# boycehbz/MvSMPLfitting

Hardware: AMD Instinct MI355X
Metric: L-BFGS closure evaluations per second (fwd+bwd, all concurrently fitted problems), 8-view 1-person 4-stage fits (higher is better)
Workload: dtype f32

## Files before the change

### mvsmplfitting_amd/csrc/closure_device.h

```cpp
#pragma once
#include <cstddef>
#include "mvfit_device.h"

namespace mvfit {

struct ObsBlock {
    float camR[MVFIT_MAX_VIEWS][9];
    float camt[MVFIT_MAX_VIEWS][3];
    float camf[MVFIT_MAX_VIEWS];
    float camc[MVFIT_MAX_VIEWS][2];
    float gt[MVFIT_MAX_VIEWS * NKP * 2];
    float wc[MVFIT_MAX_VIEWS * NKP];
    float gt3d[NKP * 3];
    float c3d[NKP];
};
struct PoseBlock {
    float theta[72];
    float R[NJ][9];
    float rod[NJ][3];
    float J[NJ][3];
    float Mj[32][12];
    float G[NJ][12];
    float A[NJ][12];
};
// ... 684 lines not shown
    for (int k = 0, item = own.first; k < own.n; ++k, item += FWD_THREADS) {
        float4 v[FWD_RPS];
        fwd_item_load(M, nc_pad, item, v);
        __builtin_amdgcn_sched_barrier(0);
        fwd_item_fma(L, nc_pad, item, v);
    }
}

__device__ __forceinline__ void keypoints_from_xs(ClosureLds& L, int tid) {
    if (tid < NKP * 3) {
        const int k = tid / 3, a = tid - 3 * k;
        float acc = 0.f;
        if (L.M.padded) {
            int si[KP_NZ];
            float wi[KP_NZ], xv[KP_NZ];
#pragma unroll
            for (int t = 0; t < KP_NZ; ++t) { si[t] = L.M.kpp_s[k][t]; wi[t] = L.M.kpp_w[k][t]; }
#pragma unroll
            for (int t = 0; t < KP_NZ; ++t) xv[t] = L.xs[3 * si[t] + a];
#pragma unroll
            for (int t = 0; t < KP_NZ; ++t) acc = fmaf(wi[t], xv[t], acc);
        } else {
            for (int t = L.M.kp_start[k]; t < L.M.kp_start[k + 1]; ++t) acc = fmaf(L.M.kp_w[t], L.xs[3 * L.M.kp_s[t] + a], acc);
        }
        if (L.M.n_skel) {
            const int j = kp_joint_of(L.M, k);
            if (j >= 0) acc = L.pose.G[j][4 * a + 3];
        }
        L.kp[k][a] = acc + L.opt.x[X_TR + a];
    }
    __syncthreads();
}

__device__ __forceinline__ void sparse_forward(const DevModel& M, ClosureLds& L, bool from_pass, int tid, bool run_chain, const FwdEarly& ev) {
    const int nc = L.M.nc, nc_pad = L.M.nc_pad;
    const int nks = fwd_slices(nc_pad, STEP_NT - 64);
    if (run_chain || !from_pass) {
        const long long t_e2 = PH_CLK();
        const int wave_t0 = __builtin_amdgcn_readfirstlane(tid);
        if (ev.wave) {
            const FwdOwner own = fwd_item_owner(nc_pad, tid - 64);
            if (own.early) fwd_item_fma(L, nc_pad, own.first, ev.v);
        }
        if (wave_t0 == 0) {
            if (run_chain) chain_forward_wave(L, tid);
            PH_T(22);
        } else if (!from_pass && !ev.wave) {
            __builtin_assume(tid >= 64);
            contraction_forward(M, L, tid - 64);
        }
        PH_W(60, 64, t_e2); PH_W(62, 448, t_e2);
        __syncthreads();
    }
    PH_T(1);
    if (tid < nc) {
        const int c = tid, s = c / 3, a = c - 3 * s;
        float4 tr = make_float4(0.f, 0.f, 0.f, 0.f);
        if (L.M.sel_sparse) {
            const float4 w4 = *reinterpret_cast<const float4*>(L.M.selw[s]);
            const unsigned jj = L.M.selj[s];
            const float wv[4] = {w4.x, w4.y, w4.z, w4.w};
            float4 av[4];
#pragma unroll
            for (int t = 0; t < 4; ++t) av[t] = *reinterpret_cast<const float4*>(&L.pose.A[(jj >> (8 * t)) & 255u][4 * a]);
#pragma unroll
            for (int t = 0; t < 4; ++t) {
                tr.x = fmaf(wv[t], av[t].x, tr.x); tr.y = fmaf(wv[t], av[t].y, tr.y);
                tr.z = fmaf(wv[t], av[t].z, tr.z); tr.w = fmaf(wv[t], av[t].w, tr.w);
            }
        } else {
#pragma unroll 8
            for (int j = 0; j < NJ; ++j) {
                const float w = L.M.wT[j][s];
                const float4 av = *reinterpret_cast<const float4*>(&L.pose.A[j][4 * a]);
                tr.x = fmaf(w, av.x, tr.x); tr.y = fmaf(w, av.y, tr.y);
                tr.z = fmaf(w, av.z, tr.z); tr.w = fmaf(w, av.w, tr.w);
            }
        }
        *reinterpret_cast<float4*>(&L.T[s][4 * a]) = tr;
        if (!from_pass) {
            float vp[3];
#pragma unroll
            for (int b = 0; b < 3; ++b) {
                float v = L.M.vt_sub[3 * s + b];
                for (int k = 0; k < nks; ++k) v += L.scratch[k * nc_pad + 3 * s + b];
                vp[b] = v;
            }
            L.vposed[c] = vp[a];
            L.xs[c] = tr.x * vp[0] + tr.y * vp[1] + tr.z * vp[2] + tr.w;
        }
    }
    __syncthreads();
    keypoints_from_xs(L, tid);
}
__device__ __forceinline__ void sparse_forward(const DevModel& M, ClosureLds& L, bool from_pass, int tid, bool run_chain = true) {
    FwdEarly none;
    sparse_forward(M, L, from_pass, tid, run_chain, none);
}

template <bool SDFW = false, bool SDFT = true>
__device__ __forceinline__ double loss_combine(const DevModel& M, ClosureLds& L, int V, const DevWeights& W, bool writer) {
    const bool use_vp = (W.flags & MVFIT_F_VPOSER) != 0;
    const bool use_gmm = !use_vp && (W.flags & MVFIT_F_PRIOR_GMM);
    const int ndw = (V * NKP + 63) >> 6;
    double l_data = 0.0;
    for (int w = 0; w < ndw; ++w) l_data += L.red_d[w];
    const bool use_3d = (W.flags & MVFIT_F_USE_3D) != 0;
    if (use_3d) l_data += L.red_d[STEP_NW];
    l_data *= (double)W.data_w2;
    const double sq = L.red_d[STEP_NW - 1], sqb = L.red_d[STEP_NW - 2], san = L.red_d[STEP_NW - 3];
    const double wp2 = (double)W.pose_w * (double)W.pose_w;
    double l_pose;
    int dropped = 0;
    if (use_vp) {
        l_pose = sq * wp2;
    } else {
        double P;
        if (use_gmm) {
            int sel = 0;
            float best = L.gmm_ll[0];
            for (int m = 1; m < M.gmm_M; ++m) if (L.gmm_ll[m] < best) { best = L.gmm_ll[m]; sel = m; }
            if (writer) L.gmm_sel = sel;
            P = (double)best;
        } else {
            P = sq;
        }
        P *= wp2;
        if ((float)P > 5e4f) { P = 0.0; dropped |= 1; }
        l_pose = P + sq * (16.0 * wp2);
    }
// ... 6 lines not shown
    if (SDFT && L.sdf_adj && W.coll_w > 0.f) {
        bool answered = true;
        if constexpr (SDFW) {
            if (L.sdf_wait_tag) {
                if (!L.sh_sdf_ok) answered = false;
                else {
                    const long long t0 = wall_clock64();
                    while (__hip_atomic_load(L.sdf_wait_tag, __ATOMIC_RELAXED, __HIP_MEMORY_SCOPE_AGENT) < L.sdf_wait_want) {
                        if (wall_clock64() - t0 > 20000000) { answered = false; break; }
                        __builtin_amdgcn_s_sleep(8);
                    }
                    if (!answered && writer) { atomicAdd(L.sdf_wait_stats, 1u); L.sh_sdf_ok = 0u; }
                }
            }
        }
        const float S = answered ? sdf_ld(&L.sdf_adj->S) : __builtin_nanf("");
        const double ws = (double)W.coll_w * (double)S;
        l_coll = ws * ws;
        sdf_fac = 2.f * W.coll_w * W.coll_w * S;
    }
    const double total = l_data + l_pose + l_shape + l_angle + l_coll;
    if (writer) {
        L.sdf_fac = sdf_fac;
        L.loss_terms[0] = (float)l_data; L.loss_terms[1] = (float)l_pose; L.loss_terms[2] = (float)l_shape;
        L.loss_terms[3] = (float)l_angle; L.loss_terms[4] = (float)l_coll; L.loss_terms[5] = (float)total;
        L.flags_dropped = dropped;
        L.total = total;
    }
    return total;
}

template <bool DEFER = false>
__device__ __forceinline__ double loss_and_keypoint_grad(const DevModel& M, ClosureLds& L, int V, const DevWeights& W,
                                         bool want_grad, int tid) {
    const bool use_vp = (W.flags & MVFIT_F_VPOSER) != 0;
    const bool use_gmm = !use_vp && (W.flags & MVFIT_F_PRIOR_GMM);
    const int wave = tid >> 6;
    const int ndata = V * NKP;
    const int ndw = (ndata + 63) >> 6;
    double part = 0.0;
    float g0 = 0.f, g1 = 0.f, g2 = 0.f;
    if (tid < ndata) {
        const int v = tid / NKP, k = tid - v * NKP;
        const float X = L.kp[k][0], Y = L.kp[k][1], Z = L.kp[k][2];
        const float* Rc = L.obs.camR[v];
        const float* tc = L.obs.camt[v];
        const float f = L.obs.camf[v];
        const float cx = L.obs.camc[v][0], cy = L.obs.camc[v][1];
        const float px = Rc[0] * X + Rc[1] * Y + Rc[2] * Z + tc[0];
        const float py = Rc[3] * X + Rc[4] * Y + Rc[5] * Z + tc[1];
        const float pz = Rc[6] * X + Rc[7] * Y + Rc[8] * Z + tc[2];
        const float ipz = 1.0f / pz;
        const float u = f * (px * ipz) + cx, w_ = f * (py * ipz) + cy;
        const float rx = L.obs.gt[tid * 2] - u, ry = L.obs.gt[tid * 2 + 1] - w_;
        const float wcf = L.obs.wc[tid];
        const float w2 = wcf * wcf;
        const float rx2 = rx * rx, ry2 = ry * ry;
        const float idx = 1.0f / (rx2 + W.rho2), idy = 1.0f / (ry2 + W.rho2);
        const float gmx = W.rho2 * (rx2 * idx), gmy = W.rho2 * (ry2 * idy);
        part = (double)(w2 * (gmx + gmy));
        if (want_grad) {
            const float gu = -w2 * W.data_w2 * (2.f * rx * W.rho2 * W.rho2 * (idx * idx));
            const float gv = -w2 * W.data_w2 * (2.f * ry * W.rho2 * W.rho2 * (idy * idy));
            const float gpx = f * gu * ipz, gpy = f * gv * ipz;
            const float gpz = -f * (gu * px + gv * py) * (ipz * ipz);
            g0 = Rc[0] * gpx + Rc[3] * gpy + Rc[6] * gpz;
            g1 = Rc[1] * gpx + Rc[4] * gpy + Rc[7] * gpz;
            g2 = Rc[2] * gpx + Rc[5] * gpy + Rc[8] * gpz;
            L.gkp_part[v][k][0] = g0; L.gkp_part[v][k][1] = g1; L.gkp_part[v][k][2] = g2;
        }
    }
    if (wave < ndw) {
        const double pd = wave64_sum(part);
        if ((tid & 63) == 0) L.red_d[wave] = pd;
        if (want_grad) {
            const float s0 = wave64_sum(g0), s1 = wave64_sum(g1), s2 = wave64_sum(g2);
            if ((tid & 63) == 0) { L.red_f[wave][0] = s0; L.red_f[wave][1] = s1; L.red_f[wave][2] = s2; }
        }
    } else if (wave == STEP_NW - 3 && (W.flags & MVFIT_F_USE_3D)) {
        const int lane = tid & 63;
        double p3 = 0.0;
        if (lane < NKP * 3) {
            const int k = lane / 3;
            const float r = L.obs.gt3d[lane] - (&L.kp[0][0])[lane];
            const float c2 = L.obs.c3d[k] * L.obs.c3d[k];
            const float id = 1.0f / (r * r + W.rho2);
            p3 = (double)(c2 * (W.rho2 * (r * r * id)));
            if (want_grad) (&L.gkp3[0][0])[lane] = -c2 * W.data_w2 * (2.f * r * W.rho2 * W.rho2 * (id * id));
        }
        const double s3 = wave64_sum(p3);
        if (lane == 0) L.red_d[STEP_NW] = s3;
    } else if (wave == STEP_NW - 1) {
        const int lane = tid & 63;
        double pp = 0.0, bb = 0.0, an = 0.0;
        if (use_vp) { if (lane < 32) { const double v = (double)L.opt.x[X_EMB + lane]; pp = v * v; } }
        else {
            { const double v = (double)L.pose.theta[3 + lane]; pp = v * v; }
            if (lane < 5) { const double v = (double)L.pose.theta[3 + 64 + lane]; pp += v * v; }
        }
        if (lane < 10) { const double v = (double)L.opt.x[X_BETAS + lane]; bb = v * v; }
        if (lane < 4) {
            const int idx = lane == 0 ? 52 : lane == 1 ? 55 : lane == 2 ? 9 : 12;
            const float sg = lane == 0 ? 1.f : -1.f;
            const float e0 = expf(sg * L.pose.theta[3 + idx]);
            an = (double)(e0 * e0);
        }
        const double spp = wave64_sum(pp), sbb = wave64_sum(bb), san = wave64_sum(an);
        if (lane == 0) { L.red_d[STEP_NW - 1] = spp; L.red_d[STEP_NW - 2] = sbb; L.red_d[STEP_NW - 3] = san; }
    }
    if (use_gmm) {
        const int Mg = M.gmm_M;
        __syncthreads();
        float* dm = L.scratch;
        for (int i = tid; i < Mg * 72; i += STEP_NT) {
            const int m = i / 72, c = i - 72 * m;
            dm[i] = c < 69 ? L.pose.theta[3 + c] - M.gmm_means[m * 69 + c] : 0.f;
        }
// ... 150 lines not shown
__device__ __forceinline__ void bwd_item_load(const DevModel& M, int nc_pad, int item, float4 (&v)[BWD_CPS]) {
    constexpr int npq = KROWS >> 2;
    const int cps = ((nc_pad >> 2) + BWD_SLICES - 1) / BWD_SLICES * 4;
    const int pq = item % npq, cs = (item / npq + (int)blockIdx.x) & (BWD_SLICES - 1);
    const int c0 = cs * cps;
    const float4* src = reinterpret_cast<const float4*>(M.pd_subT) + pq;
#pragma unroll
    for (int r = 0; r < BWD_CPS; ++r) {
        const int c = min(c0 + r, nc_pad - 1);
        if (r < BWD_SMPL_CPS || r < cps) v[r] = src[(size_t)c * npq];
    }
}

__device__ __forceinline__ void bwd_item_fma(ClosureLds& L, int nc_pad, int item, const float4 (&v)[BWD_CPS]) {
    constexpr int npq = KROWS >> 2;
    const int cps = ((nc_pad >> 2) + BWD_SLICES - 1) / BWD_SLICES * 4;
    const int pq = item % npq, cs = (item / npq + (int)blockIdx.x) & (BWD_SLICES - 1);
    const int c0 = cs * cps;
    float4 acc0 = make_float4(0.f, 0.f, 0.f, 0.f), acc1 = acc0;
#pragma unroll
    for (int r = 0; r < BWD_CPS; r += 2) {
        if (r < cps) {
            const float g0 = L.gvp[c0 + r], g1 = L.gvp[c0 + r + 1];
            acc0.x = fmaf(g0, v[r].x, acc0.x); acc0.y = fmaf(g0, v[r].y, acc0.y);
            acc0.z = fmaf(g0, v[r].z, acc0.z); acc0.w = fmaf(g0, v[r].w, acc0.w);
            acc1.x = fmaf(g1, v[r + 1].x, acc1.x); acc1.y = fmaf(g1, v[r + 1].y, acc1.y);
            acc1.z = fmaf(g1, v[r + 1].z, acc1.z); acc1.w = fmaf(g1, v[r + 1].w, acc1.w);
        }
    }
    float4* dst = reinterpret_cast<float4*>(L.scratch + cs * KROWS + 4 * pq);
    *dst = make_float4(acc0.x + acc1.x, acc0.y + acc1.y, acc0.z + acc1.z, acc0.w + acc1.w);
}

template <bool REMOTE = false, bool DEFER = false, bool SDFW = false, bool SDFT = true>
__device__ __forceinline__ void closure_backward(const DevModel& M, ClosureLds& L, int V, const DevWeights& W, int tid) {
    const bool use_vp = (W.flags & MVFIT_F_VPOSER) != 0;
    const int ns = L.M.ns, nc = L.M.nc, nc_pad = L.M.nc_pad;
    static_assert(32 * NS_STRIDE * 4 <= sizeof(ModelLds), "a 16-lane row of every thread reads inside the image");
    const bool e6_cells = L.M.e6_cells != 0, n_skel = L.M.n_skel != 0;
    const uint2 e6_cw = reinterpret_cast<const uint2*>(reinterpret_cast<const char*>(&L.M) + (tid >> 4) * (NS_STRIDE * 4))[tid & 15];
    __syncthreads();
    if constexpr (DEFER) {
        static_assert(NC_MAX + NJ * 3 <= STEP_NT - 64, "E5's threads leave the last wave free");
        if (tid >= STEP_NT - 64) loss_combine<SDFW, SDFT>(M, L, V, W, tid == STEP_NT - 64);
    }
    if (tid < nc_pad) {
        float v = 0.f;
        if (tid < nc) {
            const int s = tid / 3, bq = tid - 3 * s;
            float gx0 = 0.f, gx1 = 0.f, gx2 = 0.f;
            if (L.M.padded) {
#pragma unroll
                for (int t = 0; t < VS_NZ; ++t) {
                    const int k = L.M.vsp_k[s][t];
                    const float w = L.M.vsp_w[s][t];
                    gx0 = fmaf(w, L.gkp[k][0], gx0); gx1 = fmaf(w, L.gkp[k][1], gx1); gx2 = fmaf(w, L.gkp[k][2], gx2);
                }
            } else {
                for (int t = L.M.vs_start[s]; t < L.M.vs_start[s + 1]; ++t) {
                    const int k = L.M.vs_k[t];
                    const float w = L.M.vs_w[t];
                    gx0 = fmaf(w, L.gkp[k][0], gx0); gx1 = fmaf(w, L.gkp[k][1], gx1); gx2 = fmaf(w, L.gkp[k][2], gx2);
                }
            }
            v = L.T[s][0 + bq] * gx0 + L.T[s][4 + bq] * gx1 + L.T[s][8 + bq] * gx2;
            L.gx[tid] = bq == 0 ? gx0 : (bq == 1 ? gx1 : gx2);
        }
        L.gvp[tid] = v;
    } else if (tid < NC_MAX) {
        L.gvp[tid] = 0.f;
    } else if (tid < NC_MAX + NJ * 3 && L.M.n_skel) {
        const int i = tid - NC_MAX, j = i / 3, a = i - 3 * j;
        float gs = 0.f;
        for (int k = 0; k < NKP; ++k) if (kp_joint_of(L.M, k) == j) gs += L.gkp[k][a];
        L.gM[j][a] = gs;
    }
    __syncthreads();
    PH_T(4);
    const float sdf_fac = SDFT ? L.sdf_fac : 0.f;
    static_assert(NJ * 16 % 64 == 0 && NJ * 16 < STEP_NT, "E6 leaves whole waves free");
#ifdef MVFIT_DEBUG_HOOKS
    const bool bwd_late = (__builtin_amdgcn_readfirstlane(L.M.stream_late) & 1) != 0;
#else
    constexpr bool bwd_late = false;
#endif
    const int wave_t0 = __builtin_amdgcn_readfirstlane(tid);
    const bool e7_early = !bwd_late && wave_t0 >= NJ * 16;
    float4 e7v[BWD_CPS];
    if (wave_t0 < NJ * 16) {
        const int j = tid >> 4, g = tid & 15;
        const int ta = min(g, 2);
        const float J0 = L.pose.J[j][0], J1 = L.pose.J[j][1], J2 = L.pose.J[j][2];
        const float G0 = L.pose.G[j][0 + ta], G4 = L.pose.G[j][4 + ta], G8 = L.pose.G[j][8 + ta];
        const float gm = L.gM[j][ta];
        float acc[12];
#pragma unroll
        for (int e = 0; e < 12; ++e) acc[e] = 0.f;
        auto add_vertex = [&acc](float w, float gx0, float gx1, float gx2, float v0, float v1, float v2) {
            const float g0 = w * gx0, g1 = w * gx1, g2 = w * gx2;
            acc[0] = fmaf(g0, v0, acc[0]); acc[1] = fmaf(g0, v1, acc[1]); acc[2] = fmaf(g0, v2, acc[2]);
            acc[3] = fmaf(g1, v0, acc[3]); acc[4] = fmaf(g1, v1, acc[4]); acc[5] = fmaf(g1, v2, acc[5]);
            acc[6] = fmaf(g2, v0, acc[6]); acc[7] = fmaf(g2, v1, acc[7]); acc[8] = fmaf(g2, v2, acc[8]);
            acc[9] = fmaf(w, gx0, acc[9]); acc[10] = fmaf(w, gx1, acc[10]); acc[11] = fmaf(w, gx2, acc[11]);
        };
        if (e6_cells) {
            float w[E6_NZ], gx[E6_NZ][3], vp[E6_NZ][3];
#pragma unroll
            for (int t = 0; t < E6_NZ; ++t) {
                const unsigned e = ((t & 2) ? e6_cw.y : e6_cw.x) >> (16 * (t & 1)) & 0xffffu;
                const int i = (int)(e & (E6_INVALID - 1)), s = i >> 2;
                const float wl = (&L.M.selw[0][0])[i];
                w[t] = (e & E6_INVALID) ? 0.f : wl;
#pragma unroll
                for (int a = 0; a < 3; ++a) { gx[t][a] = L.gx[3 * s + a]; vp[t][a] = L.vposed[3 * s + a]; }
            }
#pragma unroll
            for (int t = 0; t < E6_NZ; ++t) add_vertex(w[t], gx[t][0], gx[t][1], gx[t][2], vp[t][0], vp[t][1], vp[t][2]);
        } else {
            for (int s = g; s < ns; s += 16)
                add_vertex(L.M.wT[j][s], L.gx[3 * s], L.gx[3 * s + 1], L.gx[3 * s + 2], L.vposed[3 * s], L.vposed[3 * s + 1], L.vposed[3 * s + 2]);
        }
#pragma unroll
        for (int e = 0; e < 12; ++e) acc[e] = row16_sum(acc[e]);
        if (g < 3) {
            if (sdf_fac != 0.f) {
#pragma unroll
                for (int e = 0; e < 12; ++e) acc[e] = fmaf(sdf_fac, sdf_ld(&L.sdf_adj->gA[j * 12 + e]), acc[e]);
            }
            auto row = [g](float r0, float r1, float r2) { return g == 0 ? r0 : (g == 1 ? r1 : r2); };
            const float ar0 = row(acc[0], acc[3], acc[6]), ar1 = row(acc[1], acc[4], acc[7]), ar2 = row(acc[2], acc[5], acc[8]);
            const float at = row(acc[9], acc[10], acc[11]);
            *reinterpret_cast<float4*>(&L.gG[j][4 * g]) =
                make_float4(fmaf(-at, J0, ar0), fmaf(-at, J1, ar1), fmaf(-at, J2, ar2), n_skel ? at + gm : at);
            L.gJ[j][g] = -fmaf(acc[11], G8, fmaf(acc[9], G0, acc[10] * G4));
        }
    }
    if (e7_early) bwd_item_load(M, nc_pad, tid - 64, e7v);
    __syncthreads();
// ... 266 lines not shown
```

### mvsmplfitting_amd/csrc/fit_kernels.hip

```cpp
#include <hip/hip_runtime.h>

#include <algorithm>
#include <utility>

#include "closure_device.h"
#include "fit_kernels.h"
namespace mvfit {

__device__ __forceinline__ int cmap(int i, bool use_vp) {
    if (!use_vp) return i;
    return i < 13 ? i : (i < 17 ? X_TR + (i - 13) : X_EMB + (i - 17));
}
__device__ __forceinline__ int dact(bool use_vp) { return use_vp ? 49 : 86; }

template <bool CALL = false>
__device__ __forceinline__ void pose_and_chain(const DevModel& M, ClosureLds& L, uint32_t flags, int tid) {
    pose_prep<CALL>(M, L, flags, tid);
    chain_forward_block(L, tid);
}

__device__ __forceinline__ void store_block16(void* dst_g, const void* src_l, int nbytes, int tid) {
    const int n = nbytes / 16;
    for (int i = tid; i < n; i += STEP_NT) reinterpret_cast<float4*>(dst_g)[i] = reinterpret_cast<const float4*>(src_l)[i];
}
// ... 26 lines not shown
    ClosureLds& L = *reinterpret_cast<ClosureLds*>(smem_raw);
    const int b = blockIdx.x, tid = threadIdx.x;
    prologue(L, M, obs + b, nullptr, nullptr, nullptr, nullptr, params + (size_t)b * DV, tid);
    __syncthreads();
    pose_and_chain(M, L, flags, tid);
    publish_pose(L, P, b, tid);
    if (full_pose && tid < 72) full_pose[(size_t)b * 72 + tid] = L.pose.theta[tid];
}

template <bool REMOTE>
__global__ __launch_bounds__(STEP_NT) void closure_kernel(DevModel M, const ObsBlock* __restrict__ obs, int nviews,
                                                          DevWeights W, DevPose P, const float* __restrict__ params,
                                                          int from_pass, float* __restrict__ loss,
                                                          float* __restrict__ grad, float* __restrict__ joints,
                                                          const SdfAdj* __restrict__ sdf_adj) {
    extern __shared__ __attribute__((aligned(16))) unsigned char smem_raw[];
    if (REMOTE && (int)blockIdx.x >= M.vps.nprob) {
        vposer_helper(M.vpt, M.vps, smem_raw, (int)blockIdx.x % M.vps.nsets, ((int)blockIdx.x - M.vps.nprob) / M.vps.nsets);
        return;
    }
    ClosureLds& L = *reinterpret_cast<ClosureLds*>(smem_raw);
    const int b = blockIdx.x, tid = threadIdx.x;
    prologue(L, M, obs + b, nullptr, nullptr, from_pass ? P.vposed_sel + (size_t)b * NC_MAX : nullptr,
             from_pass ? P.xs_sel + (size_t)b * NC_MAX : nullptr, params + (size_t)b * DV, tid, sdf_adj ? sdf_adj + b : nullptr);
    __syncthreads();
    FwdEarly ev;
    ev.wave = fwd_early_wave(L, from_pass == 0, tid);
    if constexpr (REMOTE) {
        pose_prep_decode_inl<true>(M, L, W.flags, tid);
        pose_prep_elems(M, L, W.flags, tid, ev);
    } else {
        pose_prep(M, L, W.flags, tid, ev);
    }
    sparse_forward(M, L, from_pass != 0, tid, true, ev);
    if constexpr (REMOTE) publish_pose(L, P, b, tid);
    const bool want_grad = grad != nullptr;
    const double total = loss_and_keypoint_grad(M, L, nviews, W, want_grad, tid);
    if (tid == 0 && loss) loss[b] = (float)total;
    if (joints && tid < NKP * 3) joints[(size_t)b * NKP * 3 + tid] = (&L.kp[0][0])[tid];
    if (want_grad) {
        closure_backward<REMOTE>(M, L, nviews, W, tid);
        if (tid < DV) grad[(size_t)b * DV + tid] = L.grad[tid];
    }
    if constexpr (REMOTE) {
        __syncthreads();
        if (tid == 0 && L.vp_remote) vps_store(vps_request_slot(M.vps), 0.f, (L.vp_seq + 1u) << 2 | VPS_BYE);
    }
}

__global__ __launch_bounds__(64) void joints_kernel(DevModel M, const float* __restrict__ verts, const float* __restrict__ Amat,
                                                    const float* __restrict__ params, float* __restrict__ joints) {
    const int b = blockIdx.x, tid = threadIdx.x;
    const ModelLds& C = *M.mlds;
    if (tid < NKP * 3) {
        const int k = tid / 3, a = tid - 3 * k;
        float s = 0.f;
        const int j = kp_joint_of(C, k);
        if (j >= 0) {
            const float* x = params + (size_t)b * DV;
            const float* A = Amat + (size_t)b * 288 + j * 12 + 4 * a;
            float J[3];
#pragma unroll
            for (int c = 0; c < 3; ++c) {
                float v = C.J_t[3 * j + c];
#pragma unroll
                for (int l = 0; l < 10; ++l) v = fmaf(C.J_S[3 * j + c][l], x[X_BETAS + l], v);
                J[c] = v;
            }
            s = A[3] + (A[0] * J[0] + A[1] * J[1] + A[2] * J[2]) + x[X_TR + a];
        } else {
// ... 30 lines not shown
    store_block16(F.opt + b, &L.opt, sizeof(OptBlock), tid);
    if (publish) {
        pose_and_chain(M, L, flags, tid);
        publish_pose(L, P, b, tid);
        store_block16(F.pose + b, &L.pose, sizeof(PoseBlock), tid);
        if (flags & MVFIT_F_VPOSER) store_block16(F.vp + b, L.vp_pre1, sizeof(VpBlock), tid);
    }
}

struct SdfService { const DevPose* P; int* gate; const unsigned* tag; int b; int round0; };
template <bool REMOTE = false, bool REUSE = false, bool LEAN = false, bool COMPACT = false, bool SDFS = false, bool ROFF = SDFS,
          bool SDFT = true>
__device__ __forceinline__ bool fit_round(const DevModel& M, ClosureLds& L, int nviews, const LbHist<float>& H,
                          bool from_pass, bool have_pose, double* stage_final, int tid,
                          LbGramLds GL = LbGramLds{nullptr, 0, 0}, float* trace = nullptr, int trace_cap = 0,
                          const AsyncRing& ring = AsyncRing{}, bool use_ring = false, int pb = 0,
                          const SdfService& sv = SdfService{nullptr, nullptr, nullptr, 0, 0}) {
    DevWeights W = L.sw[L.sh_stage];
    W.flags = __builtin_amdgcn_readfirstlane(W.flags);
    if constexpr (LEAN) {
        W.flags &= ~(uint32_t)(MVFIT_F_VPOSER | MVFIT_F_PRIOR_GMM | MVFIT_F_USE_3D);
        __builtin_assume((W.flags & (MVFIT_F_VPOSER | MVFIT_F_PRIOR_GMM | MVFIT_F_USE_3D)) == 0);
    }
    const LbOpts& O = L.opts;
    const bool use_vp = (W.flags & MVFIT_F_VPOSER) != 0;
    PH_T0();
    FwdEarly ev;
    ev.wave = fwd_early_wave(L, !from_pass && !have_pose, tid);
    if (!have_pose) {
        pose_prep_decode_inl<REMOTE>(M, L, W.flags, tid);
        pose_prep_elems(M, L, W.flags, tid, ev);
    }
    PH_T(0);
    sparse_forward(M, L, from_pass, tid, !have_pose, ev);
    PH_T(2);
    const unsigned a_round = use_ring ? (unsigned)(L.opt.lbS.n_closure - (ROFF ? sv.round0 : 0)) : 0u;
    const int a_slot = use_ring ? (int)(a_round % (unsigned)ring.nslots) : 0;
    if (use_ring) publish_pose_async(L, ring, a_slot, a_round, pb, tid);
    bool sdf_round = false;
    if constexpr (SDFS) {
        sdf_round = use_ring && L.sdf_adj != nullptr && W.coll_w > 0.f;
        if (use_ring) publish_sdf_request(L, *sv.P, sv.gate, sv.b, sdf_round ? 1 : 0, tid);
        if (sdf_round) publish_tag(ring, a_slot, pb, a_round, tid);
        if (tid == 0) {
            L.sdf_wait_tag = sdf_round ? sv.tag + sv.b : nullptr;
            L.sdf_wait_want = a_round + 1u;
            L.sdf_wait_stats = ring.stats + 3;
        }
    }
    loss_and_keypoint_grad<true>(M, L, nviews, W, true, tid);
    PH_T(3);
    closure_backward<REMOTE, true, SDFS, SDFT>(M, L, nviews, W, tid);
    const double total = L.total;
    if (trace) {
        const int k = L.opt.lbS.n_closure;
        if (k < trace_cap) {
            if (tid < DV) trace[(size_t)k * (DV + 1) + tid] = L.opt.x[tid];
            if (tid == 0) trace[(size_t)k * (DV + 1) + DV] = (float)total;
        }
    }
    if (use_ring && !sdf_round) publish_tag(ring, a_slot, pb, a_round, tid);
    PH_T(8);
    float gnew[LB_EPL], xt[LB_EPL];
    const int D = dact(use_vp);
    if (tid < 64) {
        PH_T(9);
#pragma unroll
        for (int e = 0; e < LB_EPL; ++e) {
            const int i = LB_EPL * tid + e;
            gnew[e] = i < D ? L.grad[cmap(i, use_vp)] : 0.f;
        }
    }
    lbfgs_round<float, STEP_NT, REUSE>(&L.opt.lbS, &L.opt.lbV[0], H, L.lbW, O, (double)(float)total, gnew, xt, tid, stage_final, [&]() {
        PH_T(10);
        if constexpr (COMPACT) lb_direction_compact<float, STEP_NT>(H, L.lbW, tid, lb_dir_forms(O));
        else lb_direction_block<float, STEP_NT>(H, L.lbW, tid, GL);
        PH_T(11); PH_ADD(15, 1);
    });
    if (tid < 64) {
#pragma unroll
        for (int e = 0; e < LB_EPL; ++e) {
            const int i = LB_EPL * tid + e;
            if (i < D) L.opt.x[cmap(i, use_vp)] = xt[e];
// ... 436 lines not shown
```

### mvsmplfitting_amd/csrc/model_layout.h

```cpp
#pragma once
#include <stdint.h>

namespace mvfit {

constexpr int NJ = 24;
constexpr int NKP = 17;
constexpr int KROWS = 224;
constexpr int KGROUPS = 28;
constexpr int TILE_V = 32;
constexpr int NS_MAX = 96;
constexpr int NS_STRIDE = 112;
constexpr int NC_MAX = NS_MAX * 3;
constexpr int KNNZ_MAX = 160;
constexpr int KP_NZ = 12;
constexpr int VS_NZ = 2;
constexpr int VPS_SLICES = 8;
constexpr int VPS_PMAX = 24;
constexpr int VPS_MAX_SETS = 16;

constexpr int E1_POSE_T = NJ * 12;
constexpr int E1_NPOSE = (NJ - 1) * 9;
constexpr int E1_WORKERS = E1_POSE_T + (KROWS - E1_NPOSE);
constexpr int E1_IDLE_T0 = 320;
static_assert(E1_WORKERS <= E1_IDLE_T0 && E1_IDLE_T0 % 64 == 0, "E1's workers leave whole waves free");
constexpr int FWD_SLICES = 8, FWD_RPS = KROWS / FWD_SLICES;
constexpr int FWD_THREADS = 512 - 64, FWD_EARLY_T0 = E1_IDLE_T0 - 64;
static_assert(FWD_EARLY_T0 + FWD_THREADS >= (NC_MAX / 4) * FWD_SLICES, "an early thread owns one item at most");
struct FwdOwner { int first, n; bool early; };
constexpr FwdOwner fwd_item_owner(int nc_pad, int t) {
    const int nitems = (nc_pad >> 2) * FWD_SLICES;
    const int n = t >= nitems ? 0 : (t + FWD_THREADS < nitems ? 2 : 1);
    return FwdOwner{t, n, n > 0 && t >= FWD_EARLY_T0};
}

struct ModelLds {
    float wT[NJ][NS_STRIDE];
    float J_t[NJ * 3];
    float J_S[NJ * 3][11];
    float vt_sub[NC_MAX];
    int sel_v[NS_MAX];
    int kp_start[NKP + 1];
    int kp_s[KNNZ_MAX];
    float kp_w[KNNZ_MAX];
    int vs_start[NS_MAX + 1];
    int vs_k[KNNZ_MAX];
    float vs_w[KNNZ_MAX];
    int kpp_s[NKP][KP_NZ];
    float kpp_w[NKP][KP_NZ];
    int vsp_k[NS_MAX][VS_NZ];
    float vsp_w[NS_MAX][VS_NZ];
    int padded;
    unsigned kp_joint[3];
    int parents[NJ];
    int nlevels;
    int level_start[NJ + 1];
    int level_joints[NJ];
    int child_start[NJ + 1];
    int child_list[NJ];
    int n_fwd, n_bwd;
    int fwd_tab[NJ][5];
    int bwd_tab[NJ][5];
    int anc_tab[5][NJ];
    int n_jump, n_skel, jpad1, jpad2;
    int ns, nc, nc_pad, pad0;
    float selw[NS_MAX][4];
    unsigned selj[NS_MAX];
    int sel_sparse, e6_cells, stream_late, spad2;
};
constexpr int E6_NZ = 4;
constexpr unsigned E6_INVALID = 0x8000u;
constexpr int E6_ROW_BYTES = 16 * E6_NZ * 2;
static_assert(E6_ROW_BYTES % 16 == 0 && E6_ROW_BYTES <= NS_STRIDE * 4 && NS_MAX * 4 <= (int)E6_INVALID, "E6 cells fit a row of wT");
static_assert(sizeof(ModelLds) % 16 == 0, "ModelLds is bulk-copied as 16-byte words");
static_assert(NKP <= 18 && NJ < 31, "kp_joint packs six 5-bit entries per word");

}
```

### mvsmplfitting_amd/csrc/model_prep.cpp

```cpp
#include "model_prep.h"

#include <math.h>
#include <algorithm>
#include <cmath>
#include <cstdarg>
#include <cstdio>
#include <cstring>

namespace mvfit {
namespace {

constexpr int NPOSE = 207;
constexpr int NBASIS = 217;

int fail(std::string& err, int code, const char* fmt, ...) {
    char buf[512];
    va_list ap;
    va_start(ap, fmt);
    vsnprintf(buf, sizeof(buf), fmt, ap);
    va_end(ap);
    err = buf;
    return code;
}

// ... 166 lines not shown
        }
    int nnz = 0;
    for (int k = 0; k < NKP; ++k) {
        G.kp_start[k] = nnz;
        for (int s = 0; s < ns; ++s) {
            const double w = ksel[(size_t)k * nv + sel[s]];
            if (w == 0.0) continue;
            if (nnz >= KNNZ_MAX) return fail(err, MVFIT_E_UNSUPPORTED, "keypoint selection has more than %d non-zeros", KNNZ_MAX);
            G.kp_s[nnz] = s; G.kp_w[nnz] = (float)w; ++nnz;
        }
    }
    G.kp_start[NKP] = nnz;
    nnz = 0;
    for (int s = 0; s < ns; ++s) {
        G.vs_start[s] = nnz;
        for (int k = 0; k < NKP; ++k) {
            const double w = ksel[(size_t)k * nv + sel[s]];
            if (w == 0.0) continue;
            G.vs_k[nnz] = k; G.vs_w[nnz] = (float)w; ++nnz;
        }
    }
    for (int s = ns; s <= NS_MAX; ++s) G.vs_start[s] = nnz;
    G.padded = 1;
    for (int k = 0; k < NKP; ++k) {
        const int n0 = G.kp_start[k], cnt = G.kp_start[k + 1] - n0;
        if (cnt > KP_NZ) G.padded = 0;
        for (int t = 0; t < KP_NZ; ++t) { G.kpp_s[k][t] = t < cnt ? G.kp_s[n0 + t] : 0; G.kpp_w[k][t] = t < cnt ? G.kp_w[n0 + t] : 0.f; }
    }
    for (int s = 0; s < NS_MAX; ++s) {
        const int n0 = G.vs_start[s], cnt = G.vs_start[s + 1] - n0;
        if (cnt > VS_NZ) G.padded = 0;
        for (int t = 0; t < VS_NZ; ++t) { G.vsp_k[s][t] = t < cnt ? G.vs_k[n0 + t] : 0; G.vsp_w[s][t] = t < cnt ? G.vs_w[n0 + t] : 0.f; }
    }
    h.tile_sel_start.assign(h.ntiles + 1, 0);
    h.tile_sel_local.assign(ns, 0);
    h.tile_sel_slot.assign(ns, 0);
    int pos = 0;
    for (int T = 0; T < h.ntiles; ++T) {
        h.tile_sel_start[T] = pos;
        for (int s = 0; s < ns; ++s)
            if (sel[s] / TILE_V == T) { h.tile_sel_local[pos] = sel[s] % TILE_V; h.tile_sel_slot[pos] = s; ++pos; }
    }
    h.tile_sel_start[h.ntiles] = pos;
    return MVFIT_OK;
}

int build_chain(const mvfit_model& m, ModelLds& G, std::string& err) {
    int depth[NJ];
    for (int j = 0; j < NJ; ++j) {
        G.parents[j] = m.parents[j];
        if (j > 0 && (m.parents[j] < 0 || m.parents[j] >= j)) return fail(err, MVFIT_E_ARG, "parents must be topologically ordered");
        depth[j] = j == 0 ? 0 : depth[m.parents[j]] + 1;
    }
    int maxd = 0;
    for (int j = 0; j < NJ; ++j) maxd = std::max(maxd, depth[j]);
    G.nlevels = maxd + 1;
    int pos = 0;
    for (int lv = 0; lv <= maxd; ++lv) {
        G.level_start[lv] = pos;
        for (int j = 0; j < NJ; ++j) if (depth[j] == lv) G.level_joints[pos++] = j;
    }
    for (int lv = maxd + 1; lv <= NJ; ++lv) G.level_start[lv] = pos;
    pos = 0;
    for (int p = 0; p < NJ; ++p) {
        G.child_start[p] = pos;
        for (int j = 1; j < NJ; ++j) if (m.parents[j] == p) G.child_list[pos++] = j;
// ... 148 lines not shown
```

### mvsmplfitting_amd/csrc/mvfit_api.hip

```cpp
#include <dlfcn.h>

#include "model_prep.h"
#include "mvfit_ctx.h"

template <typename T>
static T* dev_upload(mvfit_ctx* c, const T* h, size_t n) {
    if (n == 0) return nullptr;
    T* d = nullptr;
    if (c->model_mem.alloc(&d, n * sizeof(T)) != hipSuccess) c->alloc_failed = true;
    else if (hipMemcpy(d, h, n * sizeof(T), hipMemcpyHostToDevice) != hipSuccess) c->upload_failed = true;
    return d;
}
template <typename T>
static T* dev_upload(mvfit_ctx* c, const std::vector<T>& h) { return dev_upload(c, h.data(), h.size()); }
template <typename D, typename T>
static const D* dev_upload_as(mvfit_ctx* c, const std::vector<T>& h) { return reinterpret_cast<const D*>(dev_upload(c, h)); }

static void upload_model(mvfit_ctx* c, const HostModel& h) {
    DevModel& M = c->M;
    c->nv = M.nv = h.nv;
    M.nv_pad = h.nv_pad;
    M.ntiles = h.ntiles;
    M.bs4 = dev_upload(c, h.bs4);
    M.bs_h2 = dev_upload_as<float4>(c, h.bs_h2);
    M.bs_scale = h.bs_scale;
    M.half_basis = h.half_basis;
    M.vt_planes = dev_upload(c, h.vt_planes);
    M.wt_tiles = dev_upload(c, h.wt_tiles);
    M.wsp_w = dev_upload_as<float4>(c, h.wsp_w);
    M.wsp_j = dev_upload_as<int4>(c, h.wsp_j);
    M.bs_vm = dev_upload(c, h.bs_vm);
    M.w_vm = dev_upload(c, h.w_vm);
    M.ns = h.ns; M.nc = h.nc; M.nc_pad = h.nc_pad;
    M.sel_v = dev_upload(c, h.sel_v);
    M.pd_sub = dev_upload(c, h.pd_sub);
    M.pd_subT = dev_upload(c, h.pd_subT);
    M.tile_sel_start = dev_upload(c, h.tile_sel_start);
    M.tile_sel_local = dev_upload(c, h.tile_sel_local);
    M.tile_sel_slot = dev_upload(c, h.tile_sel_slot);
    {
        std::vector<unsigned char> img(sizeof(ModelLds) + NJ * E6_ROW_BYTES, 0);
        ModelLds lds = h.lds;
        if (debug_hook("MVFIT_E6_DENSE") != 0) lds.e6_cells = 0;
        if (debug_hook("MVFIT_BWD_STREAM_LATE") != 0) lds.stream_late |= 1;
        if (debug_hook("MVFIT_FWD_STREAM_LATE") != 0) lds.stream_late |= 2;
        memcpy(img.data(), &lds, sizeof(ModelLds));
        memcpy(img.data() + sizeof(ModelLds), h.e6_cells.data(), std::min<size_t>(h.e6_cells.size() * 2, NJ * E6_ROW_BYTES));
        M.mlds = reinterpret_cast<const ModelLds*>(dev_upload(c, img));
    }
    M.vp_w1 = dev_upload(c, h.vp_w1); M.vp_b1 = dev_upload(c, h.vp_b1);
    M.vp_w2 = dev_upload(c, h.vp_w2); M.vp_b2 = dev_upload(c, h.vp_b2);
    M.vp_w3 = dev_upload(c, h.vp_w3); M.vp_b3 = dev_upload(c, h.vp_b3);
    M.vp_w1T = dev_upload(c, h.vp_w1T); M.vp_w2T = dev_upload(c, h.vp_w2T); M.vp_w3T = dev_upload(c, h.vp_w3T);
    M.vpt.tw2 = dev_upload_as<float4>(c, h.vp_tw2);
    M.vpt.tw3 = dev_upload_as<float4>(c, h.vp_tw3);
    M.vpt.w1T = M.vp_w1T; M.vpt.b1 = M.vp_b1; M.vpt.b2 = M.vp_b2;
    c->has_vposer = h.has_vposer;
    c->gmm_M = M.gmm_M = h.gmm_M;
    M.gmm_means = dev_upload(c, h.gmm_means);
    M.gmm_prec = dev_upload(c, h.gmm_prec);
    M.gmm_precT = dev_upload(c, h.gmm_precT);
    M.gmm_lognw = dev_upload(c, h.gmm_lognw);
    c->d_faces = dev_upload(c, h.faces);
    c->d_vf_ptr = dev_upload(c, h.vf_ptr);
    c->d_vf_idx = dev_upload(c, h.vf_idx);
    c->num_faces = h.num_faces;
}

void mvfit::drop_graph(mvfit_ctx* c) {
    if (c->round_graph) { hipGraphExecDestroy(c->round_graph); c->round_graph = nullptr; }
    c->graph_key.clear();
}

extern "C" const char* mvfit_last_error(const mvfit_ctx* ctx) { return ctx ? ctx->err.c_str() : "null ctx"; }

FitPlanIn mvfit::plan_inputs(const mvfit_ctx* c) {
    FitPlanIn in;
    in.B = c->B; in.n_cu = c->n_cu; in.ntiles = c->M.ntiles;
// ... 668 lines not shown
```

### mvsmplfitting_amd/csrc/mvfit_ctx.h

```cpp
#pragma once
#include <hip/hip_runtime.h>

#include <algorithm>
#include <cmath>
#include <cstdarg>
#include <cstdio>
#include <cstdlib>
#include <cstring>
#include <string>
#include <utility>
#include <vector>

#include "dev_mem.h"
#include "fit_kernels.h"
#include "fit_plan.h"
#include "launchers.h"
#include "round_term.h"
#include "scan_loss.h"
#include "silhouette.h"
#include "term_mix.h"
#include "vertex_target.h"

using namespace mvfit;

// ... 62 lines not shown
    SilTerm silt;
    ScanState scan;
    ScanTerm scant;
    VtxTargets vt;
    TermMix mix;
    DevModel M{};
    bool upload_failed = false, alloc_failed = false;
    int nv = 0;
    bool has_vposer = false;
    int gmm_M = 0;
    int32_t *d_faces = nullptr, *d_vf_ptr = nullptr, *d_vf_idx = nullptr;
    int num_faces = 0;
    unsigned long long* vps_mem = nullptr;
    size_t vps_words = 0;
    unsigned vps_stats[3] = {0, 0, 0};
    DevProblems Q{};
    int B = 0, Bpad = 0, V = 0;
    ProblemBufs pb;
    DevPose P{};
    FitBuffers F{};
    bool has_joints3d = false;
    hipEvent_t ev_done[2] = {nullptr, nullptr};
    AsyncRing ring{};
    hipStream_t pass_stream = nullptr;
    hipEvent_t ev_batch[4] = {nullptr, nullptr, nullptr, nullptr}, ev_init = nullptr;
    unsigned async_stats[4] = {0, 0, 0, 0};
    mvfit_options opt{};
    int n_cu = 0;
    int resident_tpw = 0;
    int h_queue0 = 0;
    bool resident_auto_off = false;
    double res_span_ms = 0.0, res_busy_ms = 0.0, res_slowest_ms = 0.0;
    int res_rounds = 0;
    float* capture_verts = nullptr;
    int capture_round = -1;
    float* trace = nullptr;
    int trace_cap = 0;
    hipGraphExec_t round_graph = nullptr;
    std::vector<unsigned char> graph_key;
    int graph_rounds = 0;
    unsigned graph_builds = 0;
    int sdf_num_faces = 0, sdf_grid = 0;
    int sdf_op_B = 0, sdf_op_F = 0;
    int sdf_op_path = 0, sdf_term_path = 0;
    bool sdf_cull_refused = false;
    Obstacles obst;
    hipEvent_t scene_copied[2] = {nullptr, nullptr};
    int scene_slot = 0;
    bool profile = false;
    std::vector<std::pair<hipEvent_t, hipEvent_t>> ev_vp, ev_step;
};

namespace mvfit {

inline int fail(mvfit_ctx* c, int code, const char* fmt, ...) {
    char buf[512];
    va_list ap;
    va_start(ap, fmt);
    vsnprintf(buf, sizeof(buf), fmt, ap);
    va_end(ap);
    if (c) c->err = buf;
    return code;
}

}

// ... 54 lines not shown
```

Measured before the change: 1.702 million.

## Compute keypoints per wave and fuse E5 vertex-gradient pass into E6

Each data wave now builds its own copy of the keypoints in scratch right after the forward skinning barrier. This replaces the shared keypoints_from_xs pass and its trailing block-wide barrier. The keypoint regressor coefficients are also prefetched before that barrier. In the deferred backward path, when the model is padded, cell-based and has no skeleton, the gradient scatter from keypoints to vertices (E5) is recomputed inside the E6 joint accumulation, which drops one barrier-separated phase. The cost is redundant arithmetic and LDS reads across waves and more register pressure from the preloaded sparse weights.

```diff
diff --git a/mvsmplfitting_amd/csrc/closure_device.h b/mvsmplfitting_amd/csrc/closure_device.h
--- a/mvsmplfitting_amd/csrc/closure_device.h
+++ b/mvsmplfitting_amd/csrc/closure_device.h
@@ -740,7 +740,61 @@
     __syncthreads();
 }
 
-__device__ __forceinline__ void sparse_forward(const DevModel& M, ClosureLds& L, bool from_pass, int tid, bool run_chain, const FwdEarly& ev) {
+struct KpEarly {
+    bool per_wave = false, wave = false;
+    int si[KP_NZ];
+    float wi[KP_NZ];
+    int padded, n_skel;
+    float tr;
+};
+__device__ __forceinline__ KpEarly kp_early(const ClosureLds& L, int V, uint32_t flags, int tid) {
+    KpEarly kq;
+#ifdef MVFIT_DEBUG_HOOKS
+    kq.per_wave = (__builtin_amdgcn_readfirstlane(L.M.stream_late) & 4) == 0;
+#else
+    kq.per_wave = true;
+#endif
+    kq.wave = kq.per_wave && kp_copy_wave(V, (flags & MVFIT_F_USE_3D) != 0, __builtin_amdgcn_readfirstlane(tid) >> 6, STEP_NW);
+    return kq;
+}
+__device__ __forceinline__ void kp_early_load(const ClosureLds& L, int tid, KpEarly& kq) {
+    const int i = min(tid & 63, NKP * 3 - 1), k = i / 3;
+#pragma unroll
+    for (int t = 0; t < KP_NZ; ++t) { kq.si[t] = L.M.kpp_s[k][t]; kq.wi[t] = L.M.kpp_w[k][t]; }
+    kq.padded = L.M.padded; kq.n_skel = L.M.n_skel;
+    kq.tr = L.opt.x[X_TR + (i - 3 * k)];
+}
+
+__device__ __forceinline__ void keypoints_wave_copy(ClosureLds& L, int tid, const KpEarly& kq, float* mine) {
+    const int lane = tid & 63;
+    if (lane < NKP * 3) {
+        const int k = lane / 3, a = lane - 3 * k;
+        float acc = 0.f;
+        if (__builtin_amdgcn_readfirstlane(kq.padded)) {
+            int si[KP_NZ];
+            float xv[KP_NZ];
+#pragma unroll
+            for (int t = 0; t < KP_NZ; ++t) { si[t] = kq.si[t]; asm volatile("" : "+v"(si[t])); }
+#pragma unroll
+            for (int t = 0; t < KP_NZ; ++t) xv[t] = L.xs[(int)__umul24((unsigned)si[t], 3u) + a];
+#pragma unroll
+            for (int t = 0; t < KP_NZ; ++t) acc = fmaf(kq.wi[t], xv[t], acc);
+        } else {
+            for (int t = L.M.kp_start[k]; t < L.M.kp_start[k + 1]; ++t) acc = fmaf(L.M.kp_w[t], L.xs[3 * L.M.kp_s[t] + a], acc);
+        }
+        if (__builtin_amdgcn_readfirstlane(kq.n_skel)) {
+            const int j = kp_joint_of(L.M, k);
+            if (j >= 0) acc = L.pose.G[j][4 * a + 3];
+        }
+        const float v = acc + kq.tr;
+        mine[lane] = v;
+        if (tid < 64) (&L.kp[0][0])[lane] = v;
+    }
+    wave_lds_fence();
+}
+
+__device__ __forceinline__ void sparse_forward(const DevModel& M, ClosureLds& L, bool from_pass, int tid, bool run_chain, const FwdEarly& ev,
+                                               KpEarly& kq) {
     const int nc = L.M.nc, nc_pad = L.M.nc_pad;
     const int nks = fwd_slices(nc_pad, STEP_NT - 64);
     if (run_chain || !from_pass) {
@@ -761,6 +815,7 @@
         __syncthreads();
     }
     PH_T(1);
+    if (kq.wave) kp_early_load(L, tid, kq);
     if (tid < nc) {
         const int c = tid, s = c / 3, a = c - 3 * s;
         float4 tr = make_float4(0.f, 0.f, 0.f, 0.f);
@@ -799,11 +854,12 @@
         }
     }
     __syncthreads();
-    keypoints_from_xs(L, tid);
+    if (!kq.per_wave) keypoints_from_xs(L, tid);
 }
 __device__ __forceinline__ void sparse_forward(const DevModel& M, ClosureLds& L, bool from_pass, int tid, bool run_chain = true) {
     FwdEarly none;
-    sparse_forward(M, L, from_pass, tid, run_chain, none);
+    KpEarly phase;
+    sparse_forward(M, L, from_pass, tid, run_chain, none, phase);
 }
 
 template <bool SDFW = false, bool SDFT = true>
@@ -876,17 +932,24 @@
 
 template <bool DEFER = false>
 __device__ __forceinline__ double loss_and_keypoint_grad(const DevModel& M, ClosureLds& L, int V, const DevWeights& W,
-                                         bool want_grad, int tid) {
+                                         bool want_grad, int tid, const KpEarly& kq) {
     const bool use_vp = (W.flags & MVFIT_F_VPOSER) != 0;
     const bool use_gmm = !use_vp && (W.flags & MVFIT_F_PRIOR_GMM);
     const int wave = tid >> 6;
     const int ndata = V * NKP;
     const int ndw = (ndata + 63) >> 6;
+    static_assert(STEP_NW * KP_COPY_STRIDE <= 8 * NC_MAX && NKP * 3 <= KP_COPY_STRIDE, "a keypoint copy per wave in the scratch");
+    const float* kpv = &L.kp[0][0];
+    if (kq.wave) {
+        float* mine = L.scratch + __builtin_amdgcn_readfirstlane(wave) * KP_COPY_STRIDE;
+        keypoints_wave_copy(L, tid, kq, mine);
+        kpv = mine;
+    }
     double part = 0.0;
     float g0 = 0.f, g1 = 0.f, g2 = 0.f;
     if (tid < ndata) {
         const int v = tid / NKP, k = tid - v * NKP;
-        const float X = L.kp[k][0], Y = L.kp[k][1], Z = L.kp[k][2];
+        const float X = kpv[3 * k], Y = kpv[3 * k + 1], Z = kpv[3 * k + 2];
         const float* Rc = L.obs.camR[v];
         const float* tc = L.obs.camt[v];
         const float f = L.obs.camf[v];
@@ -926,7 +989,7 @@
         double p3 = 0.0;
         if (lane < NKP * 3) {
             const int k = lane / 3;
-            const float r = L.obs.gt3d[lane] - (&L.kp[0][0])[lane];
+            const float r = L.obs.gt3d[lane] - kpv[lane];
             const float c2 = L.obs.c3d[k] * L.obs.c3d[k];
             const float id = 1.0f / (r * r + W.rho2);
             p3 = (double)(c2 * (W.rho2 * (r * r * id)));
@@ -1143,6 +1206,12 @@
     *dst = make_float4(acc0.x + acc1.x, acc0.y + acc1.y, acc0.z + acc1.z, acc0.w + acc1.w);
 }
 
+__device__ __forceinline__ float e5_gvp(float t0, float t4, float t8, float gx0, float gx1, float gx2) {
+#pragma clang fp contract(off)
+    const float p0 = gx0 * t0, p2 = gx2 * t8;
+    return fmaf(gx1, t4, p0) + p2;
+}
+
 template <bool REMOTE = false, bool DEFER = false, bool SDFW = false, bool SDFT = true>
 __device__ __forceinline__ void closure_backward(const DevModel& M, ClosureLds& L, int V, const DevWeights& W, int tid) {
     const bool use_vp = (W.flags & MVFIT_F_VPOSER) != 0;
@@ -1150,11 +1219,46 @@
     static_assert(32 * NS_STRIDE * 4 <= sizeof(ModelLds), "a 16-lane row of every thread reads inside the image");
     const bool e6_cells = L.M.e6_cells != 0, n_skel = L.M.n_skel != 0;
     const uint2 e6_cw = reinterpret_cast<const uint2*>(reinterpret_cast<const char*>(&L.M) + (tid >> 4) * (NS_STRIDE * 4))[tid & 15];
+    bool fused = false;
+    if constexpr (DEFER && !SDFT) {
+        fused = e6_cells && L.M.e5_in_e6 != 0;
+#ifdef MVFIT_DEBUG_HOOKS
+        if (__builtin_amdgcn_readfirstlane(L.M.stream_late) & 8) fused = false;
+#endif
+    }
+    float e6_kw[E6_NZ][VS_NZ];
+    int e6_kk[E6_NZ][VS_NZ];
+    if (fused && __builtin_amdgcn_readfirstlane(tid) < NJ * 16) {
+#pragma unroll
+        for (int t = 0; t < E6_NZ; ++t) {
+            const unsigned e = ((t & 2) ? e6_cw.y : e6_cw.x) >> (16 * (t & 1)) & 0xffffu;
+            const int s = (int)(e & (E6_INVALID - 1)) >> 2;
+#pragma unroll
+            for (int u = 0; u < VS_NZ; ++u) { e6_kk[t][u] = L.M.vsp_k[s][u]; e6_kw[t][u] = L.M.vsp_w[s][u]; }
+        }
+    }
     __syncthreads();
     if constexpr (DEFER) {
         static_assert(NC_MAX + NJ * 3 <= STEP_NT - 64, "E5's threads leave the last wave free");
         if (tid >= STEP_NT - 64) loss_combine<SDFW, SDFT>(M, L, V, W, tid == STEP_NT - 64);
     }
+    if (fused) {
+        PH_T(4);
+        if (tid < nc) {
+            const int s = tid / 3, bq = tid - 3 * s;
+            float gx0 = 0.f, gx1 = 0.f, gx2 = 0.f;
+#pragma unroll
+            for (int t = 0; t < VS_NZ; ++t) {
+                const int k = L.M.vsp_k[s][t];
+                const float w = L.M.vsp_w[s][t];
+                gx0 = fmaf(w, L.gkp[k][0], gx0); gx1 = fmaf(w, L.gkp[k][1], gx1); gx2 = fmaf(w, L.gkp[k][2], gx2);
+            }
+            L.gvp[tid] = e5_gvp(L.T[s][0 + bq], L.T[s][4 + bq], L.T[s][8 + bq], gx0, gx1, gx2);
+            L.gx[tid] = bq == 0 ? gx0 : (bq == 1 ? gx1 : gx2);
+        } else if (tid < NC_MAX) {
+            L.gvp[tid] = 0.f;
+        }
+    } else {
     if (tid < nc_pad) {
         float v = 0.f;
         if (tid < nc) {
@@ -1188,6 +1292,7 @@
     }
     __syncthreads();
     PH_T(4);
+    }
     const float sdf_fac = SDFT ? L.sdf_fac : 0.f;
     static_assert(NJ * 16 % 64 == 0 && NJ * 16 < STEP_NT, "E6 leaves whole waves free");
 #ifdef MVFIT_DEBUG_HOOKS
@@ -1214,7 +1319,31 @@
             acc[6] = fmaf(g2, v0, acc[6]); acc[7] = fmaf(g2, v1, acc[7]); acc[8] = fmaf(g2, v2, acc[8]);
             acc[9] = fmaf(w, gx0, acc[9]); acc[10] = fmaf(w, gx1, acc[10]); acc[11] = fmaf(w, gx2, acc[11]);
         };
-        if (e6_cells) {
+        if (fused) {
+            float w[E6_NZ], vp[E6_NZ][3], gk[E6_NZ][VS_NZ][3];
+#pragma unroll
+            for (int t = 0; t < E6_NZ; ++t) {
+                const unsigned e = ((t & 2) ? e6_cw.y : e6_cw.x) >> (16 * (t & 1)) & 0xffffu;
+                const int i = (int)(e & (E6_INVALID - 1)), s = i >> 2;
+                const float wl = (&L.M.selw[0][0])[i];
+                w[t] = (e & E6_INVALID) ? 0.f : wl;
+#pragma unroll
+                for (int u = 0; u < VS_NZ; ++u)
+#pragma unroll
+                    for (int a = 0; a < 3; ++a) gk[t][u][a] = L.gkp[e6_kk[t][u]][a];
+#pragma unroll
+                for (int a = 0; a < 3; ++a) vp[t][a] = L.vposed[3 * s + a];
+            }
+#pragma unroll
+            for (int t = 0; t < E6_NZ; ++t) {
+                float gx0 = 0.f, gx1 = 0.f, gx2 = 0.f;
+#pragma unroll
+                for (int u = 0; u < VS_NZ; ++u) {
+                    gx0 = fmaf(e6_kw[t][u], gk[t][u][0], gx0); gx1 = fmaf(e6_kw[t][u], gk[t][u][1], gx1); gx2 = fmaf(e6_kw[t][u], gk[t][u][2], gx2);
+                }
+                add_vertex(w[t], gx0, gx1, gx2, vp[t][0], vp[t][1], vp[t][2]);
+            }
+        } else if (e6_cells) {
             float w[E6_NZ], gx[E6_NZ][3], vp[E6_NZ][3];
 #pragma unroll
             for (int t = 0; t < E6_NZ; ++t) {
diff --git a/mvsmplfitting_amd/csrc/fit_kernels.hip b/mvsmplfitting_amd/csrc/fit_kernels.hip
--- a/mvsmplfitting_amd/csrc/fit_kernels.hip
+++ b/mvsmplfitting_amd/csrc/fit_kernels.hip
@@ -82,10 +82,11 @@
     } else {
         pose_prep(M, L, W.flags, tid, ev);
     }
-    sparse_forward(M, L, from_pass != 0, tid, true, ev);
+    KpEarly kq = kp_early(L, nviews, W.flags, tid);
+    sparse_forward(M, L, from_pass != 0, tid, true, ev, kq);
     if constexpr (REMOTE) publish_pose(L, P, b, tid);
     const bool want_grad = grad != nullptr;
-    const double total = loss_and_keypoint_grad(M, L, nviews, W, want_grad, tid);
+    const double total = loss_and_keypoint_grad(M, L, nviews, W, want_grad, tid, kq);
     if (tid == 0 && loss) loss[b] = (float)total;
     if (joints && tid < NKP * 3) joints[(size_t)b * NKP * 3 + tid] = (&L.kp[0][0])[tid];
     if (want_grad) {
@@ -182,7 +183,8 @@
         pose_prep_elems(M, L, W.flags, tid, ev);
     }
     PH_T(0);
-    sparse_forward(M, L, from_pass, tid, !have_pose, ev);
+    KpEarly kq = kp_early(L, nviews, W.flags, tid);
+    sparse_forward(M, L, from_pass, tid, !have_pose, ev, kq);
     PH_T(2);
     const unsigned a_round = use_ring ? (unsigned)(L.opt.lbS.n_closure - (ROFF ? sv.round0 : 0)) : 0u;
     const int a_slot = use_ring ? (int)(a_round % (unsigned)ring.nslots) : 0;
@@ -198,7 +200,7 @@
             L.sdf_wait_stats = ring.stats + 3;
         }
     }
-    loss_and_keypoint_grad<true>(M, L, nviews, W, true, tid);
+    loss_and_keypoint_grad<true>(M, L, nviews, W, true, tid, kq);
     PH_T(3);
     closure_backward<REMOTE, true, SDFS, SDFT>(M, L, nviews, W, tid);
     const double total = L.total;
diff --git a/mvsmplfitting_amd/csrc/model_layout.h b/mvsmplfitting_amd/csrc/model_layout.h
--- a/mvsmplfitting_amd/csrc/model_layout.h
+++ b/mvsmplfitting_amd/csrc/model_layout.h
@@ -33,6 +33,14 @@
     return FwdOwner{t, n, n > 0 && t >= FWD_EARLY_T0};
 }
 
+constexpr int KP_COPY_STRIDE = 64;
+constexpr int kp_data_waves(int nviews) { return (nviews * NKP + 63) >> 6; }
+constexpr bool kp_copy_wave(int nviews, bool use_3d, int wave, int nwaves = 8) {
+    return wave < kp_data_waves(nviews) || (use_3d && wave == nwaves - 3);
+}
+
+constexpr bool e5_in_e6_model(int e6_cells, int padded, int n_skel) { return e6_cells != 0 && padded != 0 && n_skel == 0; }
+
 struct ModelLds {
     float wT[NJ][NS_STRIDE];
     float J_t[NJ * 3];
@@ -65,7 +73,7 @@
     int ns, nc, nc_pad, pad0;
     float selw[NS_MAX][4];
     unsigned selj[NS_MAX];
-    int sel_sparse, e6_cells, stream_late, spad2;
+    int sel_sparse, e6_cells, stream_late, e5_in_e6;
 };
 constexpr int E6_NZ = 4;
 constexpr unsigned E6_INVALID = 0x8000u;
diff --git a/mvsmplfitting_amd/csrc/model_prep.cpp b/mvsmplfitting_amd/csrc/model_prep.cpp
--- a/mvsmplfitting_amd/csrc/model_prep.cpp
+++ b/mvsmplfitting_amd/csrc/model_prep.cpp
@@ -222,6 +222,7 @@
         if (cnt > VS_NZ) G.padded = 0;
         for (int t = 0; t < VS_NZ; ++t) { G.vsp_k[s][t] = t < cnt ? G.vs_k[n0 + t] : 0; G.vsp_w[s][t] = t < cnt ? G.vs_w[n0 + t] : 0.f; }
     }
+    G.e5_in_e6 = e5_in_e6_model(G.e6_cells, G.padded, G.n_skel) ? 1 : 0;
     h.tile_sel_start.assign(h.ntiles + 1, 0);
     h.tile_sel_local.assign(ns, 0);
     h.tile_sel_slot.assign(ns, 0);
diff --git a/mvsmplfitting_amd/csrc/mvfit_api.hip b/mvsmplfitting_amd/csrc/mvfit_api.hip
--- a/mvsmplfitting_amd/csrc/mvfit_api.hip
+++ b/mvsmplfitting_amd/csrc/mvfit_api.hip
@@ -15,6 +15,10 @@
 static T* dev_upload(mvfit_ctx* c, const std::vector<T>& h) { return dev_upload(c, h.data(), h.size()); }
 template <typename D, typename T>
 static const D* dev_upload_as(mvfit_ctx* c, const std::vector<T>& h) { return reinterpret_cast<const D*>(dev_upload(c, h)); }
+
+#ifdef MVFIT_DEBUG_HOOKS
+extern "C" __attribute__((visibility("default"))) int mvfit_debug_model_flags(const mvfit_ctx* ctx) { return ctx ? ctx->debug_model_flags : -1; }
+#endif
 
 static void upload_model(mvfit_ctx* c, const HostModel& h) {
     DevModel& M = c->M;
@@ -41,9 +45,14 @@
     {
         std::vector<unsigned char> img(sizeof(ModelLds) + NJ * E6_ROW_BYTES, 0);
         ModelLds lds = h.lds;
-        if (debug_hook("MVFIT_E6_DENSE") != 0) lds.e6_cells = 0;
+        if (debug_hook("MVFIT_E6_DENSE") != 0) lds.e6_cells = lds.e5_in_e6 = 0;
         if (debug_hook("MVFIT_BWD_STREAM_LATE") != 0) lds.stream_late |= 1;
         if (debug_hook("MVFIT_FWD_STREAM_LATE") != 0) lds.stream_late |= 2;
+        if (debug_hook("MVFIT_KP_PHASE") != 0) lds.stream_late |= 4;
+        if (debug_hook("MVFIT_E5_PHASE") != 0) lds.stream_late |= 8;
+#ifdef MVFIT_DEBUG_HOOKS
+        c->debug_model_flags = (lds.padded ? 1 : 0) | (lds.e6_cells ? 2 : 0) | (lds.e5_in_e6 ? 4 : 0) | lds.stream_late << 8;
+#endif
         memcpy(img.data(), &lds, sizeof(ModelLds));
         memcpy(img.data() + sizeof(ModelLds), h.e6_cells.data(), std::min<size_t>(h.e6_cells.size() * 2, NJ * E6_ROW_BYTES));
         M.mlds = reinterpret_cast<const ModelLds*>(dev_upload(c, img));
diff --git a/mvsmplfitting_amd/csrc/mvfit_ctx.h b/mvsmplfitting_amd/csrc/mvfit_ctx.h
--- a/mvsmplfitting_amd/csrc/mvfit_ctx.h
+++ b/mvsmplfitting_amd/csrc/mvfit_ctx.h
@@ -118,6 +118,9 @@
     bool resident_auto_off = false;
     double res_span_ms = 0.0, res_busy_ms = 0.0, res_slowest_ms = 0.0;
     int res_rounds = 0;
+#ifdef MVFIT_DEBUG_HOOKS
+    int debug_model_flags = 0;
+#endif
     float* capture_verts = nullptr;
     int capture_round = -1;
     float* trace = nullptr;
```

Result: no change. 1.717 million (median of 6 runs) (+0.9%).
